# letitiabanana/PnP-OVSS

Measured on AMD Instinct MI355X. Metric: images/sec (336^2, drop_iter=4, blur+CRF), higher is better.
Workload: dtype bf16x3

## Files before the change

pnp-ovss_amd/csrc/engine.hip:

```cpp
#include <hip/hip_runtime.h>

#include <cmath>
#include <cstdarg>
#include <cstring>
#include <map>
#include <memory>
#include <string>
#include <utility>
#include <vector>

#include "../../include/pnp_hip.h"
#include "common.h"
#include "kernels.h"

using namespace pnp;

namespace {

struct Buf {
    void* p = nullptr;
    size_t bytes = 0;
};

struct Weight {
// ... 1569 lines not shown
        if (hist && p.d_gt) KCHK(e, confusion_hist(lab, p.d_gt, p.d_desc, p.d_label_off, hist, n_class, p.B, p.maxHW, s));
    }
    return PNP_OK;
}


extern "C" int pnp_get_buffer(pnp_engine* e, const char* name, void** d_ptr, size_t* bytes) {
    if (!e || !name || !d_ptr || !bytes) return PNP_ERR_ARG;
    const std::string n(name);
    const size_t B = e->c.max_batch, L = e->c.max_text_len;
    auto& p = e->post;
    auto set = [&](void* ptr, size_t b) { *d_ptr = ptr; *bytes = b; return PNP_OK; };
    if (n == "image_embeds") return set(e->emb32, B * e->N * (size_t)e->D * 4);
    if (n == "image_embeds_t") return set(e->embT.hi, B * e->N * (size_t)e->D * e->esz);
    if (n == "x") return set(e->x, B * e->N * (size_t)e->D * 4);
    if (n == "P") return set(e->ta[e->grad_layer >= 0 ? e->grad_layer : e->SL].Pc, B * e->nh * L * (size_t)e->Nst * 4);
    if (n == "dP") return set(e->dPc, B * e->nh * L * (size_t)e->Nst * 4);
    if (n == "text_hidden") return set(e->ta[e->TL - 1].h_out, B * L * (size_t)e->H * 4);
    if (n == "h_last") return set(e->ta[e->TL - 1].h_out, B * L * (size_t)e->H * 4);
    if (n == "dropped") return set(e->dropped, B * (size_t)e->PP);
    if (n == "P_last" && e->ta[e->TL - 1].Pc) return set(e->ta[e->TL - 1].Pc, B * e->nh * L * (size_t)e->Nst * 4);
    if (n == "Kt" && e->Kt) return set(e->Kt, (size_t)(e->TL - e->SL - 1) * e->H * B * e->Npad * e->esz);
    if (n == "Vt") return set(e->Vt, (size_t)e->TL * e->H * B * e->Npad * e->esz);
    if (n == "dq_xattn") return set(e->dqc, B * L * (size_t)e->H * e->esz);
    if (n == "dctx_xattn") return set(e->dctxc, B * L * (size_t)e->H * e->esz);
    if (p.reserved) {
        const size_t mk = (size_t)p.max_total_pix * p.maxK * 4;
        const size_t mq = (size_t)p.max_total_pix * p.maxKp * 4;
        if (n == "merged") return set(p.merged, (size_t)p.maxB * p.maxK * e->PP * 4);
        if (n == "maps") return set(p.maps_in_2 ? p.maps2 : p.maps, mk);
        if (n == "maps_pre_blur") return set(p.maps, mk);
        if (n == "unary") return set(p.unary, mq);
        if (n == "crf_q") return set(p.Q, mq);
        if (n == "crf_idbase_gauss") return set(p.lat[0].idbase, ((size_t)p.maxB + 1) * 4);
        if (n == "crf_idbase_bilateral") return set(p.lat[1].idbase, ((size_t)p.maxB + 1) * 4);
        if (n == "crf_norm_gauss") return set(p.norm[0], (size_t)p.max_total_pix * 4);
        if (n == "crf_norm_bilateral") return set(p.norm[1], (size_t)p.max_total_pix * 4);
        if (n == "crf_offset_gauss") return set(p.lat[0].offset, (size_t)p.max_total_pix * 3 * 4);
        if (n == "crf_offset_bilateral") return set(p.lat[1].offset, (size_t)p.max_total_pix * 6 * 4);
        if (n == "crf_nbr8_gauss") return set(p.lat[0].nbr8, (size_t)(p.lat[0].D1 / 2) * p.lat[0].cap * sizeof(CrfNbr8));
        if (n == "crf_nbr8_bilateral") return set(p.lat[1].nbr8, (size_t)(p.lat[1].D1 / 2) * p.lat[1].cap * sizeof(CrfNbr8));
    }
    return fail(e, PNP_ERR_ARG, "unknown buffer %s", name);
}

extern "C" size_t pnp_allocated_bytes(const pnp_engine* e) { return e ? e->alloc_bytes : 0; }

extern "C" int pnp_profile_enable(pnp_engine* e, int32_t on) {
    if (!e) return PNP_ERR_ARG;
    if (!e->gemm_prof) {
        if (!on) {
            e->crf_prof.on = false;
            return PNP_OK;
        }
        e->gemm_prof = new GemmProfile();
    }
    GemmProfile& pf = *e->gemm_prof;
    pf.on = on != 0;
    pf.period = on > 1 ? on : 1;
    pf.seq = 0;
    pf.used = 0;
    pf.launches = 0;
    pf.flops = 0;
    e->crf_prof.on = on != 0;
    e->crf_prof.used = 0;
    e->crf_prof.launches = 0;
    e->crf_prof.work = 0;
    e->crf_prof.lattice = 0;
    return PNP_OK;
}

extern "C" int pnp_profile_read_stage(pnp_engine* e, int32_t stage, int64_t* launches, double* work, double* ms) {
    if (!e || !launches || !work || !ms) return PNP_ERR_ARG;
    if (stage == 0) return pnp_profile_read(e, launches, work, ms);
    if (stage != 1 && stage != 2) return fail(e, PNP_ERR_ARG, "unknown profile stage %d", stage);
    auto& pf = e->crf_prof;
    double total = 0;
    for (int i = 0; i < pf.used; i++) {
        HIPCHK(e, hipEventSynchronize(pf.ev1[i]));
        float t = 0;
        HIPCHK(e, hipEventElapsedTime(&t, pf.ev0[i], pf.ev1[i]));
        total += t;
    }
    *launches = pf.launches;
    *work = stage == 1 ? pf.work : pf.lattice;
    *ms = total;
    return PNP_OK;
}

extern "C" int pnp_profile_read(pnp_engine* e, int64_t* launches, double* flops, double* ms) {
    if (!e || !launches || !flops || !ms) return PNP_ERR_ARG;
    if (!e->gemm_prof) {
        *launches = 0; *flops = 0; *ms = 0;
        return PNP_OK;
    }
    GemmProfile& pf = *e->gemm_prof;
    double total = 0;
    for (int i = 0; i < pf.used; i++) {
        HIPCHK(e, hipEventSynchronize(pf.ev1[i]));
        float t = 0;
        HIPCHK(e, hipEventElapsedTime(&t, pf.ev0[i], pf.ev1[i]));
        total += t;
    }
    *launches = pf.launches;
    *flops = pf.flops;
    *ms = total;
    return PNP_OK;
}

extern "C" int pnp_op_gemm(int32_t bf, const void* d_A, int32_t lda, const void* d_B, int32_t ldb, int32_t M, int32_t N,
                           int32_t K, const float* d_bias, const float* d_resid, int32_t ldr, float* d_out_f32, int32_t ldo,
                           int32_t gelu, void* stream) {
    GemmArgs g = G_(d_A, lda, d_B, ldb, M, N, K);
    g.bias = d_bias; g.resid = d_resid; g.ldr = ldr; g.out_f32 = d_out_f32; g.ldo = ldo;
    g.mode = gelu ? GEMM_EPI_GELU : GEMM_EPI_LINEAR;
    return gemm_nt(bf, g, (hipStream_t)stream);
}

extern "C" int pnp_op_gemm_ex(int32_t bf, const void* d_A, int32_t lda, const void* d_B, int32_t ldb, int32_t M, int32_t N,
                              int32_t K, const float* d_bias, const float* d_resid, int32_t ldr, float* d_out_f32, int32_t ldo,
                              void* d_out_t, int32_t ldo_t, int32_t mode, void* stream) {
    GemmArgs g = G_(d_A, lda, d_B, ldb, M, N, K);
    g.bias = d_bias; g.resid = d_resid; g.ldr = ldr; g.out_f32 = d_out_f32; g.ldo = ldo; g.out_t = d_out_t; g.ldo_t = ldo_t;
    g.mode = mode ? GEMM_EPI_GELU : GEMM_EPI_LINEAR;
    return gemm_nt(bf, g, (hipStream_t)stream);
}

extern "C" int pnp_op_split(const float* d_in, void* d_hi, void* d_lo, int64_t n, void* stream) {
    if (!d_in || !d_hi || !d_lo || n <= 0) return PNP_ERR_ARG;
    return split_f32(d_in, d_hi, d_lo, (size_t)n, (hipStream_t)stream);
}

extern "C" int pnp_op_gemm_x3(const void* d_A_hi, const void* d_A_lo, int32_t lda, const void* d_B_hi, const void* d_B_lo,
                              int32_t ldb, int32_t M, int32_t N, int32_t K, const float* d_bias, int32_t bias_on_rows,
                              const float* d_resid, int32_t ldr, float* d_out_f32, int32_t ldo, void* d_out_hi, void* d_out_lo,
                              int32_t ldo_t, int32_t gelu, int32_t col_div, int32_t col_pad, void* stream) {
    if (!d_A_hi || !d_A_lo || !d_B_hi || !d_B_lo) return PNP_ERR_ARG;
    GemmArgs g = G_(d_A_hi, lda, d_B_hi, ldb, M, N, K);
    g.A_lo = d_A_lo; g.B_lo = d_B_lo;
    g.bias = d_bias; g.bias_on_rows = bias_on_rows; g.resid = d_resid; g.ldr = ldr; g.out_f32 = d_out_f32; g.ldo = ldo;
    g.out_t = d_out_hi; g.out_lo = d_out_lo; g.ldo_t = ldo_t; g.col_div = col_div; g.col_pad = col_pad;
    g.mode = gelu ? GEMM_EPI_GELU : GEMM_EPI_LINEAR;
    g.sk = streamk_mode() ? streamk_ws_default() : nullptr;
    return gemm_nt(1, g, (hipStream_t)stream);
}

extern "C" int pnp_set_tuning(const char* key, int32_t value) {
    if (!key) return PNP_ERR_ARG;
    if (!strcmp(key, "streamk")) {
        if (value < 0 || value > 2) return PNP_ERR_ARG;
        set_streamk_mode(value);
        return PNP_OK;
    }
    if (!strcmp(key, "text_rows")) {
        if (value < 0 || value > 4) return PNP_ERR_ARG;
        set_text_rows(value);
        return PNP_OK;
    }
    return PNP_ERR_ARG;
}

extern "C" int pnp_streamk_status(pnp_engine* e, int64_t* launches, uint32_t* gave_up) {
    if (!launches || !gave_up) return PNP_ERR_ARG;
    StreamKWs* ws = e ? &e->sk_ws : streamk_ws_default();
    *launches = ws ? ws->launches : 0;
    *gave_up = 0;
    if (!ws || !ws->part) return PNP_OK;
    if (e) HIPCHK(e, hipSetDevice(e->c.device));
    if (hipDeviceSynchronize() != hipSuccess) return PNP_ERR_HIP;
    return streamk_ws_timeouts(ws, gave_up);
}

extern "C" int pnp_op_gemm_x3a(const float* d_A, int32_t lda, const void* d_B_hi, const void* d_B_lo, int32_t ldb, int32_t M,
                               int32_t N, int32_t K, const float* d_bias, const float* d_resid, int32_t ldr, float* d_out_f32,
                               int32_t ldo, int32_t mode, float* d_aux, int32_t ld_aux, void* stream) {
    if (!d_A || !d_B_hi || !d_B_lo || !d_out_f32 || mode < 0 || mode > 2) return PNP_ERR_ARG;
    GemmArgs g = G_(d_A, lda, d_B_hi, ldb, M, N, K);
    g.B_lo = d_B_lo; g.a_f32 = 1;
    g.bias = d_bias; g.resid = d_resid; g.ldr = ldr; g.out_f32 = d_out_f32; g.ldo = ldo;
    g.mode = mode; g.aux = d_aux; g.ld_aux = ld_aux;
    return gemm_nt(0, g, (hipStream_t)stream);
}

extern "C" int pnp_op_gemm_tokcols(int32_t bf, const void* d_A, int32_t lda, const void* d_B, int32_t ldb, int32_t M, int32_t N,
                                   int32_t K, const float* d_bias_rows, void* d_out_t, int32_t ldo_t, int32_t col_div,
                                   int32_t col_pad, void* stream) {
    if (!d_out_t || col_div < 0 || (col_div > 0 && col_pad < col_div)) return PNP_ERR_ARG;
    GemmArgs g = G_(d_A, lda, d_B, ldb, M, N, K);
    g.bias = d_bias_rows; g.bias_on_rows = 1; g.out_t = d_out_t; g.ldo_t = ldo_t; g.col_div = col_div; g.col_pad = col_pad;
    return gemm_nt(bf, g, (hipStream_t)stream);
}

extern "C" int pnp_op_gemm_args(int32_t bf, const void* d_A, int32_t lda, const void* d_B, int32_t ldb, int32_t M, int32_t N,
                                int32_t K, const float* d_bias, int32_t bias_on_rows, const float* d_resid, int32_t ldr,
                                float* d_out_f32, int32_t ldo, void* d_out_t, int32_t ldo_t, int32_t mode, float* d_aux,
                                int32_t ld_aux, int32_t row_div, int32_t col_div, int32_t col_pad, void* stream) {
    if (!d_A || !d_B || (!d_out_f32 && !d_out_t) || M <= 0 || N <= 0 || K <= 0 || lda < K || ldb < K) return PNP_ERR_ARG;
    if (mode < 0 || mode > 2 || (mode == GEMM_EPI_GELU_GRAD && !d_aux)) return PNP_ERR_ARG;
    if (row_div < 0 || col_div < 0 || (col_div > 0 && col_pad < col_div)) return PNP_ERR_ARG;
    GemmArgs g = G_(d_A, lda, d_B, ldb, M, N, K);
    g.bias = d_bias; g.bias_on_rows = bias_on_rows ? 1 : 0; g.resid = d_resid; g.ldr = ldr;
    g.out_f32 = d_out_f32; g.ldo = ldo; g.out_t = d_out_t; g.ldo_t = ldo_t;
    g.mode = mode; g.aux = d_aux; g.ld_aux = ld_aux; g.row_div = row_div; g.col_div = col_div; g.col_pad = col_pad;
    return gemm_nt(bf ? 1 : 0, g, (hipStream_t)stream);
}

extern "C" int pnp_op_vit_attention(int32_t bf, const void* d_qk, int32_t ld_qk, int32_t D, const void* d_vt, int32_t ld_vt,
                                    int32_t n_pad, void* d_ctx, int32_t B, int32_t heads, int32_t N, float scale, void* stream) {
    if (!d_qk || !d_vt || !d_ctx || B <= 0 || heads <= 0 || N <= 0) return PNP_ERR_ARG;
    return vit_attention(bf, d_qk, ld_qk, D, d_vt, ld_vt, n_pad, d_ctx, B, heads, N, scale, (hipStream_t)stream);
}

extern "C" int pnp_op_vit_attention_x3(const void* d_qkv_hi, const void* d_qkv_lo, int32_t ld_qkv, int32_t D, void* d_ctx_hi,
                                       void* d_ctx_lo, int32_t B, int32_t heads, int32_t N, float scale, void* stream) {
    if (B <= 0 || heads <= 0 || N <= 0 || ld_qkv < 3 * D) return PNP_ERR_ARG;
    return vit_attention_x3(d_qkv_hi, d_qkv_lo, ld_qkv, D, d_ctx_hi, d_ctx_lo, B, heads, N, scale, (hipStream_t)stream);
}

extern "C" int pnp_op_layernorm(const float* d_x, const float* d_w, const float* d_b, float eps, int32_t rows, int32_t D,
                                float* d_y, void* stream) {
    return layernorm(0, d_x, d_w, d_b, eps, rows, D, d_y, nullptr, nullptr, nullptr, (hipStream_t)stream);
}

extern "C" int pnp_op_xattn(int32_t bf16, int32_t mode, const void* d_nat, int32_t ld_nat, const void* d_tr, int32_t ld_tr,
                            int32_t n_pad, const void* d_x, int32_t ldx, void* d_out, int32_t ldo, float* d_probs,
                            int32_t n_stride, int32_t B, int32_t L, int32_t N, int32_t heads, void* stream) {
    if (!d_nat || !d_x || !d_probs || mode < 0 || mode > 2 || (mode != 2 && (!d_tr || !d_out))) return PNP_ERR_ARG;
    if (B <= 0 || L <= 0 || N <= 0 || heads <= 0) return PNP_ERR_ARG;
    return xattn(bf16, mode, d_nat, ld_nat, d_tr, ld_tr, n_pad, d_x, ldx, d_out, ldo, d_probs, n_stride, B, L, N, heads,
                 (hipStream_t)stream);
}

extern "C" int pnp_op_text_self_attn(int32_t bf16, const void* d_qkv, const int64_t* d_mask, int32_t ld_mask, void* d_ctx,
                                     float* d_probs, float* d_scratch, int32_t B, int32_t L, int32_t H, void* stream) {
    if (!d_qkv || !d_mask || !d_ctx || B <= 0 || L <= 0 || H <= 0 || ld_mask < L) return PNP_ERR_ARG;
    return text_self_attn(bf16, d_qkv, d_mask, ld_mask, d_ctx, d_probs, d_scratch, B, L, H, (hipStream_t)stream);
}

extern "C" int pnp_op_text_self_attn_bwd(int32_t bf16, const void* d_qkv, const float* d_dctx, const float* d_probs,
                                         float* d_ds_scratch, void* d_dqkv, int32_t B, int32_t L, int32_t H, void* stream) {
    if (!d_qkv || !d_dctx || !d_probs || !d_ds_scratch || !d_dqkv || B <= 0 || L <= 0 || H <= 0) return PNP_ERR_ARG;
    return text_self_attn_bwd(bf16, d_qkv, d_dctx, d_probs, d_ds_scratch, d_dqkv, B, L, H, (hipStream_t)stream);
}

extern "C" int pnp_op_layernorm_ex(int32_t bf16, const float* d_x, const float* d_w, const float* d_b, float eps, int32_t rows,
                                   int32_t D, float* d_y, void* d_yt, void* d_yt_lo, float* d_xhat, float* d_rstd, void* stream) {
    if (!d_x || !d_w || !d_b || rows <= 0 || D <= 0 || (d_yt_lo && !d_yt)) return PNP_ERR_ARG;
    return layernorm(bf16, d_x, d_w, d_b, eps, rows, D, d_y, d_yt, d_xhat, d_rstd, (hipStream_t)stream, d_yt_lo);
}

extern "C" int pnp_op_layernorm_bwd(int32_t bf16, const float* d_dy, const float* d_w, const float* d_xhat, const float* d_rstd,
                                    int32_t rows, int32_t D, float* d_dx, void* d_dxt, void* stream) {
    if (!d_dy || !d_w || !d_xhat || !d_rstd || rows <= 0 || D <= 0) return PNP_ERR_ARG;
    return layernorm_bwd(bf16, d_dy, d_w, d_xhat, d_rstd, rows, D, d_dx, d_dxt, (hipStream_t)stream);
}

extern "C" int pnp_op_text_embed(const int64_t* d_ids, int32_t ld_ids, const float* d_word, const float* d_pos, float* d_out,
                                 int32_t B, int32_t L, int32_t H, int32_t enc_id, int32_t vocab, void* stream) {
    if (!d_ids || !d_word || !d_pos || !d_out || B <= 0 || L <= 0 || H <= 0 || H % 4 || vocab <= 0 || ld_ids < L || enc_id >= vocab)
        return PNP_ERR_ARG;
    return text_embed(d_ids, ld_ids, d_word, d_pos, d_out, B, L, H, enc_id, vocab, (hipStream_t)stream);
}

extern "C" int pnp_op_itm_head(const float* d_hlast, const float* d_w, const float* d_bias, float* d_logits, int32_t B, int32_t L,
                               int32_t H, void* stream) {
    if (!d_hlast || !d_w || !d_bias || !d_logits || B <= 0 || L <= 0 || H <= 0) return PNP_ERR_ARG;
    return itm_head(d_hlast, d_w, d_bias, d_logits, B, L, H, (hipStream_t)stream);
}

extern "C" int pnp_op_itm_grad_seed(const float* d_w, float* d_dh, int32_t B, int32_t L, int32_t H, void* stream) {
    if (!d_w || !d_dh || B <= 0 || L <= 0 || H <= 0) return PNP_ERR_ARG;
    return itm_grad_seed(d_w, d_dh, B, L, H, (hipStream_t)stream);
}

extern "C" int pnp_op_patchify(int32_t bf16, const float* d_img, const uint8_t* d_dropped, void* d_out, int32_t B, int32_t S,
                               int32_t P, void* stream) {
    if (!d_img || !d_out || B <= 0 || P <= 0 || S != P * 16) return PNP_ERR_ARG;
    return patchify(bf16, d_img, d_dropped, d_out, B, S, P, (hipStream_t)stream);
}

extern "C" int pnp_op_cls_rows(const float* d_cls, const float* d_pos, float* d_x, int32_t B, int32_t N, int32_t D, void* stream) {
    if (!d_cls || !d_pos || !d_x || B <= 0 || N <= 0 || D <= 0) return PNP_ERR_ARG;
    return cls_rows(d_cls, d_pos, d_x, B, N, D, (hipStream_t)stream);
}

extern "C" int pnp_dbg_gemm_stamps(uint64_t* host_out, int32_t max_blocks) {
    return gemm_read_stamps((unsigned long long*)host_out, max_blocks);
}

extern "C" int pnp_preprocess_images(const uint8_t* d_rgb, const pnp_pre_image* d_desc, int32_t B, int32_t S, int32_t max_H,
                                     const int32_t* d_coef, uint8_t* d_tmp, const float* mean3, const float* std3,
                                     float* d_out, void* stream) {
    if (!d_rgb || !d_desc || !d_coef || !d_tmp || !mean3 || !std3 || !d_out) return PNP_ERR_ARG;
    static_assert(sizeof(pnp_pre_image) == 40, "pnp_pre_image layout is part of the ABI");
    return preprocess_images(d_rgb, d_desc, B, S, max_H, d_coef, d_tmp, mean3, std3, d_out, (hipStream_t)stream);
}

extern "C" int pnp_jpeg_decode(const uint8_t* d_data, const pnp_jpeg_image* d_images, const pnp_jpeg_tables* d_tables,
                               const pnp_jpeg_segment* d_segments, int32_t n_images, int32_t n_segments, uint8_t* d_clean,
                               int32_t* d_seg_bits, int16_t* d_coef, int64_t coef_elems, uint8_t* d_planes, uint8_t* d_rgb,
                               int32_t max_blocks_per_image, int32_t max_pixels_per_image, int32_t* d_err, void* stream) {
    if (!d_data || !d_images || !d_tables || !d_segments || !d_clean || !d_seg_bits || !d_coef || !d_planes || !d_rgb || !d_err ||
        coef_elems <= 0)
        return PNP_ERR_ARG;
    static_assert(sizeof(pnp_jpeg_image) == sizeof(JpegImage) && sizeof(pnp_jpeg_tables) == sizeof(JpegTables) &&
                      sizeof(pnp_jpeg_segment) == sizeof(JpegSegment), "JPEG descriptor layouts are part of the ABI");
// ... 33 lines not shown
```

pnp-ovss_amd/csrc/kernels.h:

```cpp
#pragma once
#include <hip/hip_runtime.h>
#include <stdint.h>
#include <stddef.h>
#include "gemm.h"

namespace pnp {

struct PostDesc {
    int H, W, K, C, has_bg, pix0;
    int Kp;
    int G, Kg;
    size_t off;
    size_t qoff;
    size_t voff[2];
};

struct alignas(16) CrfEntry {
    uint32_t pixel;
    float w;
    float nr;
    uint32_t pad;
};

struct alignas(16) CrfNbr8 {
    int ia, id;
    int pa, pd;
    int aa, ad;
    int da, dd;
};

struct CrfLattice {
    int D1;
    int which;
    size_t cap;
    float* bary;
    uint32_t* vals;
    CrfEntry* ent;
    int* offset;
    int* seg_start;
    int* seg_lo;
    int* seg_hi;
    uint64_t* ukeys;
    int* idbase;
    int* n1;
    int* n2;
    CrfNbr8* nbr8;
};

int patchify(int bf, const float* img, const uint8_t* dropped, void* out, int B, int S, int P, hipStream_t s);
int cls_rows(const float* cls, const float* pos, float* x, int B, int N, int D, hipStream_t s);
int layernorm(int bf, const float* x, const float* w, const float* b, float eps, int rows, int D, float* y, void* yt,
              float* xhat, float* rstd, hipStream_t s, void* yt_lo = nullptr);
int vit_attention(int bf, const void* qk, int ld_qk, int D, const void* vt, int ld_vt, int Npad, void* ctx, int B,
                  int H, int N, float scale, hipStream_t s, void* ctx_lo = nullptr);

int vit_attention_x3(const void* qkv_hi, const void* qkv_lo, int ld_qk, int D, void* ctx_hi, void* ctx_lo, int B, int H, int N,
                     float scale, hipStream_t s);

int text_embed(const int64_t* ids, int ld_ids, const float* word, const float* pos, float* out, int B, int L, int H,
               int enc_id, int vocab, hipStream_t s);
int text_self_attn(int bf, const void* qkv, const int64_t* mask, int ld_mask, void* ctx, float* probs, float* scratch, int B, int L,
                   int H, hipStream_t s);
void set_text_rows(int n);
int text_self_attn_bwd(int bf, const void* qkv, const float* dctx, const float* probs, float* ds_scratch, void* dqkv,
                       int B, int L, int H, hipStream_t s);
int xattn(int bf, int mode, const void* a1, int ld1, const void* a2t, int ld2, int Npad, const void* x, int ldx,
          void* out, int ldo, float* pbuf, int Nst, int B, int L, int N, int nheads, hipStream_t s);
int layernorm_bwd(int bf, const float* dy, const float* w, const float* xhat, const float* rstd, int rows, int D,
                  float* dx, void* dxt, hipStream_t s);
int itm_head(const float* hlast, const float* w, const float* bias, float* logits, int B, int L, int H, hipStream_t s);
int itm_grad_seed(const float* w, float* dh, int B, int L, int H, hipStream_t s);
int cast_f32(int bf, const float* in, void* out, size_t n, hipStream_t s);
int split_f32(const float* in, void* hi, void* lo, size_t n, hipStream_t s);

int l2_normalize_rows(float* x, int rows, int E, float eps, hipStream_t s);
int itc_similarity(const float* img, const float* txt, float* sim, int B, int T, int E, hipStream_t s);
int cast_rows_bf16(const float* in, int ld_in, void* out, int rows, int K, hipStream_t s);

int gradcam_gather(const float* P, const float* dP, const int64_t* mask, int ld_mask, float* out, int B, int nheads,
                   int head, int L, int Nst, int PP, hipStream_t s);
int drop_step(const float* G, float* g0, float* agg, uint8_t* dropped, int32_t* picks, int iter, int B, int T, int PP,
              int npick, int max_picks, hipStream_t s);
int merge_tokens(const float* src, const int32_t* cls_off, const int32_t* tok_idx, const int32_t* cls_div,
                 const int32_t* img_cls_off, float* out, int B, int T, int PP, int Cmax, hipStream_t s);
int threshold_maps(const float* merged, const int32_t* img_cls_off, float* out, float threshold, int B, int PP, int Cmax,
                   hipStream_t s);
int upsample_maps(const float* src, const PostDesc* desc, float* maps, int B, int P, int Cmax, int maxHW, hipStream_t s);
int minmax_normalize(float* maps, const PostDesc* desc, float* stats, int B, int Kmax, int maxHW, int class_channels_only,
                     hipStream_t s);
int background_channel(float* maps, const PostDesc* desc, int B, int maxHW, hipStream_t s);
int blur_maps(const float* in, float* tmp, float* out, const PostDesc* desc, const double* wts, const int32_t* wt_off,
              int B, int Kmax, int maxH, int maxW, int max_radius, hipStream_t s);
int preprocess_images(const uint8_t* rgb, const void* desc, int B, int S, int max_H, const int32_t* coef, uint8_t* tmp,
                      const float* mean3, const float* std3, float* out, hipStream_t s);
int unary_from_maps(const float* maps, const PostDesc* desc, float* unary, int B, int maxHW, int max_kp, int group, hipStream_t s);
int argmax_remap(const float* q, const PostDesc* desc, const int32_t* lut, int lut_stride, uint8_t* labels,
                 const size_t* label_off, int pixel_major, int group, int B, int maxHW, hipStream_t s);
int confusion_hist(const uint8_t* labels, const float* gt, const PostDesc* desc, const size_t* label_off,
                   unsigned long long* hist, int n_class, int B, int maxHW, hipStream_t s);

struct JpegImage {
    int64_t data_off;
    int64_t coef_off[3];
    int64_t plane_off[3];
    int64_t rgb_off;
    int32_t data_len, H, W, ncomp, hmax, vmax, mcux, mcuy;
    int32_t h[3], v[3], tq[3], td[3], ta[3], bx[3], by[3];
    int32_t tab, pad[2];
};
struct JpegTables {
    uint8_t counts[4][16];
    uint8_t vals[4][256];
    int32_t quant[4][64];
};
struct JpegSegment {
    int64_t byte_off;
    int64_t clean_off;
    int32_t image, mcu0, nmcu;
    int32_t raw_len;
    int32_t clean_cap;
    int32_t sub_bits;
    int32_t pad[2];
};
int jpeg_decode(const uint8_t* d_data, const JpegImage* d_imgs, const JpegTables* d_tabs, const JpegSegment* d_segs, int n_images,
                int n_segments, uint8_t* d_clean, int* d_seg_bits, int16_t* d_coef, size_t coef_elems, uint8_t* d_planes, uint8_t* d_rgb,
                int max_blocks, int max_pixels, int* d_err, hipStream_t s);

size_t sort_temp_bytes(size_t n);
int radix_sort_pairs(uint64_t* keys_in, uint64_t* keys_out, uint32_t* vals_in, uint32_t* vals_out, size_t n, int begin_bit, int end_bit,
                     const size_t* seg_off, int nseg, void* temp, size_t temp_bytes, hipStream_t s);
int device_scan_i32(const int* in, int* out, size_t n, bool inclusive, void* temp, size_t temp_bytes, hipStream_t s);
size_t crf_sort_temp_bytes(size_t max_entries, int max_images);
int crf_build_lattice(int D, const CrfLattice& L, const PostDesc* d_imgs, const PostDesc* h_imgs, const uint8_t* d_rgb, float sxy, float srgb,
                      int B, size_t ent_total, int max_pixels,
                      uint64_t* keys_a, uint64_t* keys_b, uint32_t* vals_a, int* head, int* incl, int* n1k, int* n2k,
                      void* temp, size_t temp_bytes, int* d_range_err, int* h_range_err, int* h_points, hipStream_t s);
int crf_lattice_norm(const CrfLattice& L, const PostDesc* d_imgs, int B, int max_pixels, size_t ent_total, float* va, float* vb,
                     float* norm_out, hipStream_t s);
int crf_filter(const CrfLattice& L, const PostDesc* d_imgs, int img0, int nimg, const float* Q,
               float* va, float* vb, const float** result, int max_kp, hipStream_t s);
struct CrfLabelOut {
    uint8_t* lab[2] = {nullptr, nullptr};
    const int32_t* lut = nullptr;
    int lut_stride = 0;
    const size_t* label_off = nullptr;
};
int crf_update(const CrfLattice& Lg, const CrfLattice& Lb, const PostDesc* d_imgs, int img0, int nimg, const float* vg,
               const float* vb, const float* norm_g, const float* norm_b, const float* unary, float* Q, float w_g,
               float w_b, int pairwise, int max_pixels, int max_kp, int groups, hipStream_t s, const CrfLabelOut& labels = CrfLabelOut());

}
```

pnp-ovss_amd/csrc/vit_kernels.hip:

```cpp
#include <stdlib.h>

#include "common.h"
#include "kernels.h"

namespace pnp {

template <typename T>
__global__ void patchify_kernel(const float* __restrict__ img, const uint8_t* __restrict__ dropped,
                                T* __restrict__ out, int B, int S, int P) {
    const int idx = blockIdx.x * blockDim.x + threadIdx.x;
    const int total = B * P * P * 3 * 16;
    if (idx >= total) return;
    const int i = idx & 15;
    const int c = (idx >> 4) % 3;
    const int m = idx / 48;
    const int b = m / (P * P), p = m - b * P * P;
    const int py = p / P, px = p - py * P;
    T* o = out + (size_t)m * 768 + c * 256 + i * 16;
    const bool drop = dropped && dropped[m];
    const float* src = img + (((size_t)b * 3 + c) * S + (py * 16 + i)) * S + px * 16;
#pragma unroll
    for (int v = 0; v < 4; v++) {
        f32x4 x = drop ? f32x4{0.f, 0.f, 0.f, 0.f} : *reinterpret_cast<const f32x4*>(src + v * 4);
#pragma unroll
// ... 219 lines not shown
    const int l32 = lane & 31, hi = lane >> 5;
    const int b = blockIdx.z, h = blockIdx.y;
    const size_t row0 = (size_t)b * N;
    const int qw = blockIdx.x * nwaves + wave;
    int qrow = qw * 32 + l32;
    const bool q_valid = qw < nqw && qrow < N;
    qrow = qrow < N ? qrow : N - 1;

    bf16x8 fq[4];
    {
        const bf16* qp = qk + (row0 + qrow) * ld_qk + h * 64 + hi * 8;
#pragma unroll
        for (int ks = 0; ks < 4; ks++) fq[ks] = *reinterpret_cast<const bf16x8*>(qp + ks * 16);
    }

    const char* kbase = reinterpret_cast<const char*>(qk + row0 * ld_qk + D + h * 64);
    const char* vbase = reinterpret_cast<const char*>(vt + row0 * ld_vt + h * 64);
    const int prow = lane >> 3, pc = lane & 7;
    auto issue_tile = [&](int t) {
        char* dst = ring[t & 1];
        for (int p = wave; p < 16; p += nwaves) {
            const int row = (p & 7) * 8 + prow;
            const int sc = pc ^ ((row >> 1) & 7);
            int key = t * 64 + row;
            key = key < N ? key : N - 1;
            const char* src = p < 8 ? kbase + (size_t)key * ld_qk * 2 + sc * 16 : vbase + (size_t)key * ld_vt * 2 + sc * 16;
            __builtin_amdgcn_global_load_lds((const __attribute__((address_space(1))) void*)src,
                                             (__attribute__((address_space(3))) void*)(dst + p * 1024), 16, 0, 0);
        }
    };

    f32x16 o[2];
#pragma unroll
    for (int i = 0; i < 2; i++)
#pragma unroll
        for (int e = 0; e < 16; e++) o[i][e] = 0.f;
    float m_run = -INFINITY, l_run = 0.f;
    const float c = scale * 1.4426950408889634f;
    const int sw = (l32 >> 1) & 7;
    const int ntiles = (N + 63) / 64;

    issue_tile(0);
    for (int t = 0; t < ntiles; t++) {
        asm volatile("s_waitcnt vmcnt(0)" ::: "memory");
        __builtin_amdgcn_s_barrier();
        if (t + 1 < ntiles) issue_tile(t + 1);
        const char* Ks = ring[t & 1];
        const char* Vs = Ks + TILE;

        bf16x8 fk[2][4];
#pragma unroll
        for (int kt = 0; kt < 2; kt++)
#pragma unroll
            for (int ks = 0; ks < 4; ks++)
                fk[kt][ks] = *reinterpret_cast<const bf16x8*>(Ks + (kt * 32 + l32) * ROWB + (((ks * 2 + hi) ^ sw) << 4));
        f32x16 s[2];
        const f32x16 zero16 = {0.f, 0.f, 0.f, 0.f, 0.f, 0.f, 0.f, 0.f, 0.f, 0.f, 0.f, 0.f, 0.f, 0.f, 0.f, 0.f};
#pragma unroll
        for (int kt = 0; kt < 2; kt++) {
            s[kt] = __builtin_amdgcn_mfma_f32_32x32x16_bf16(fk[kt][0], fq[0], zero16, 0, 0, 0);
#pragma unroll
            for (int ks = 1; ks < 4; ks++) s[kt] = __builtin_amdgcn_mfma_f32_32x32x16_bf16(fk[kt][ks], fq[ks], s[kt], 0, 0, 0);
        }
        if (t == ntiles - 1 && (N & 63)) {
#pragma unroll
            for (int kt = 0; kt < 2; kt++)
#pragma unroll
                for (int e = 0; e < 16; e++) {
                    const int key = t * 64 + kt * 32 + (e >> 2) * 8 + hi * 4 + (e & 3);
                    if (key >= N) s[kt][e] = -INFINITY;
                }
        }
        float mx;
        asm("v_max3_f32 %0, %1, %2, %3" : "=v"(mx) : "v"(s[0][0]), "v"(s[0][1]), "v"(s[0][2]));
#pragma unroll
        for (int e = 3; e + 1 < 16; e += 2) asm("v_max3_f32 %0, %1, %2, %3" : "=v"(mx) : "v"(mx), "v"(s[0][e]), "v"(s[0][e + 1]));
        asm("v_max3_f32 %0, %1, %2, %3" : "=v"(mx) : "v"(mx), "v"(s[0][15]), "v"(s[1][0]));
#pragma unroll
        for (int e = 1; e + 1 < 16; e += 2) asm("v_max3_f32 %0, %1, %2, %3" : "=v"(mx) : "v"(mx), "v"(s[1][e]), "v"(s[1][e + 1]));
        asm("v_max3_f32 %0, %1, %2, %3" : "=v"(mx) : "v"(mx), "v"(s[1][15]), "v"(m_run));
        const float m_new = fmaxf(mx, __shfl_xor(mx, 32, 64));
        {
            const float alpha = __builtin_amdgcn_exp2f((m_run - m_new) * c);
#pragma unroll
            for (int i = 0; i < 2; i++) o[i] *= alpha;
            l_run *= alpha;
            m_run = m_new;
        }
        const float mc = -m_run * c;
        bf16x8 fp[4];
#pragma unroll
        for (int kt = 0; kt < 2; kt++)
#pragma unroll
            for (int e = 0; e < 16; e++) {
                const float p = __builtin_amdgcn_exp2f(fmaf(s[kt][e], c, mc));
                l_run += p;
                fp[kt * 2 + (e >> 3)][e & 7] = (bf16)p;
            }
        const int grp_d = ((lane >> 4) & 1) * 16, tq = (lane >> 2) & 3, tp = lane & 3;
#pragma unroll
        for (int j = 0; j < 4; j++)
#pragma unroll
            for (int dt = 0; dt < 2; dt++) {
                typedef __attribute__((ext_vector_type(4))) short s16x4;
                s16x4 part[2];
#pragma unroll
                for (int u = 0; u < 2; u++) {
                    const int key = 16 * j + 8 * u + 4 * hi + tq;
                    const int col = dt * 32 + grp_d + 4 * tp;
                    const char* a = Vs + key * ROWB + ((((col >> 3)) ^ ((key >> 1) & 7)) << 4) + (col & 7) * 2;
                    part[u] = __builtin_amdgcn_ds_read_tr16_b64_v4i16((__attribute__((address_space(3))) s16x4*)a);
                }
                const bf16x4 lo = __builtin_bit_cast(bf16x4, part[0]), hh = __builtin_bit_cast(bf16x4, part[1]);
                const bf16x8 fv = {lo[0], lo[1], lo[2], lo[3], hh[0], hh[1], hh[2], hh[3]};
                o[dt] = __builtin_amdgcn_mfma_f32_32x32x16_bf16(fv, fp[j], o[dt], 0, 0, 0);
            }
    }
    l_run += __shfl_xor(l_run, 32, 64);
    if (q_valid) {
        const float inv = 1.0f / l_run;
        bf16* op = ctx + (row0 + qrow) * D + h * 64 + hi * 4;
#pragma unroll
        for (int dt = 0; dt < 2; dt++)
#pragma unroll
            for (int g4 = 0; g4 < 4; g4++) {
                const bf16x4 pk = {(bf16)(o[dt][g4 * 4] * inv), (bf16)(o[dt][g4 * 4 + 1] * inv), (bf16)(o[dt][g4 * 4 + 2] * inv),
                                   (bf16)(o[dt][g4 * 4 + 3] * inv)};
                *reinterpret_cast<bf16x4*>(op + dt * 32 + g4 * 8) = pk;
            }
    }
}

#ifdef PNP_DEV
__device__ unsigned long long* g_attn_stamps = nullptr;
__device__ int g_attn_ablate = 0;
extern "C" int pnp_dev_attn_ablate(int on) {
    return hipMemcpyToSymbol(HIP_SYMBOL(g_attn_ablate), &on, sizeof(on)) == hipSuccess ? PNP_OK : PNP_ERR_HIP;
}
extern "C" int pnp_dev_attn_stamps(unsigned long long* d_buf) {
    return hipMemcpyToSymbol(HIP_SYMBOL(g_attn_stamps), &d_buf, sizeof(d_buf)) == hipSuccess ? PNP_OK : PNP_ERR_HIP;
}
#define PNP_ATTN_STAMP(k)                                                                                       \
    do {                                                                                                        \
        if (stamps && lane == 0) {                                                                              \
            __builtin_amdgcn_sched_barrier(0);                                                                  \
            stamps[((size_t)wave * ntiles + t) * 6 + (k)] = __builtin_readcyclecounter();                       \
            __builtin_amdgcn_sched_barrier(0);                                                                  \
        }                                                                                                       \
    } while (0)
#else
#define PNP_ATTN_STAMP(k) do {} while (0)
#endif

__global__ __launch_bounds__(768) void vit_attn32_x3_kernel(const bf16* __restrict__ qk, const bf16* __restrict__ qk_lo, int ld_qk, int D,
                                                            const bf16* __restrict__ vt, const bf16* __restrict__ vt_lo, int ld_vt,
                                                            bf16* __restrict__ ctx, bf16* __restrict__ ctx_lo, int N, float scale, int nqw) {
    constexpr int ROWB = 128, TILE = 64 * ROWB;
    __shared__ __attribute__((aligned(16))) char ring[2][4 * TILE];

    const int tid = threadIdx.x, lane = tid & 63, wave = __builtin_amdgcn_readfirstlane(tid >> 6);
    const int nwaves = blockDim.x >> 6;
    const int l32 = lane & 31, hi = lane >> 5;
    const int b = blockIdx.z, h = blockIdx.y;
    const size_t row0 = (size_t)b * N;
    const int qw = blockIdx.x * nwaves + wave;
    int qrow = qw * 32 + l32;
    const bool q_valid = qw < nqw && qrow < N;
    qrow = qrow < N ? qrow : N - 1;

    bf16x8 fq[4], fql[4];
    {
        const size_t off = (row0 + qrow) * ld_qk + h * 64 + hi * 8;
#pragma unroll
        for (int ks = 0; ks < 4; ks++) {
            fq[ks] = *reinterpret_cast<const bf16x8*>(qk + off + ks * 16);
            fql[ks] = *reinterpret_cast<const bf16x8*>(qk_lo + off + ks * 16);
        }
    }
    const size_t koff = (row0 * ld_qk + D + h * 64) * 2, voff = (row0 * ld_vt + h * 64) * 2;
    const uint64_t k0 = reinterpret_cast<uint64_t>(qk) + koff;
    const uint64_t d_klo = reinterpret_cast<uint64_t>(qk_lo) + koff - k0;
    const uint64_t d_v = reinterpret_cast<uint64_t>(vt) + voff - k0;
    const uint64_t d_vlo = reinterpret_cast<uint64_t>(vt_lo) + voff - k0;
    const int prow = lane >> 3, pc = lane & 7;
    const uint32_t sc_even = (uint32_t)(pc ^ ((prow >> 1) & 7)) << 4, sc_odd = (uint32_t)(pc ^ ((4 + (prow >> 1)) & 7)) << 4;
    auto issue_tile = [&](int t) {
        for (int p = wave; p < 32; p += nwaves) {
            const uint64_t m_v = 0ull - (uint64_t)((p >> 3) & 1), m_lo = 0ull - (uint64_t)(p >> 4);
            const uint64_t d = (m_v & m_lo & d_vlo) | (m_v & ~m_lo & d_v) | (~m_v & m_lo & d_klo);
            const uint32_t ld2 = ((uint32_t)ld_qk + ((uint32_t)m_v & (uint32_t)(ld_vt - ld_qk))) * 2u;
            int rs = t * 64 + (p & 7) * 8;
#ifdef PNP_DEV
            if (g_attn_ablate) rs = (p & 7) * 8;
#endif
            rs = rs < N - 1 ? rs : N - 1;
            const char* const sbase = reinterpret_cast<const char*>(k0 + d + (uint64_t)((uint32_t)rs * ld2));
            int lr = rs + prow;
            lr = (lr < N ? lr : N - 1) - rs;
            const uint32_t loff = (uint32_t)lr * ld2 + ((p & 1) ? sc_odd : sc_even);
            const uint32_t lds = (uint32_t)(uintptr_t)(__attribute__((address_space(3))) char*)(ring[t & 1] + p * 1024);
            const uint64_t sb = reinterpret_cast<uint64_t>(sbase);
            const uint64_t sbu = ((uint64_t)(uint32_t)__builtin_amdgcn_readfirstlane((int)(sb >> 32)) << 32) |
                                 (uint32_t)__builtin_amdgcn_readfirstlane((int)(uint32_t)sb);
            asm volatile("s_mov_b32 m0, %2\n\ts_nop 0\n\tglobal_load_lds_dwordx4 %0, %1" ::"v"(loff), "s"(sbu),
                         "s"(__builtin_amdgcn_readfirstlane((int)lds))
                         : "memory");
        }
    };

    f32x16 o[2];
#pragma unroll
    for (int i = 0; i < 2; i++)
#pragma unroll
        for (int e = 0; e < 16; e++) o[i][e] = 0.f;
    float m_run = -INFINITY, l_run = 0.f;
    const float c = scale * 1.4426950408889634f;
    const int sw = (l32 >> 1) & 7;
    const int ntiles = (N + 63) / 64;

#ifdef PNP_DEV
    unsigned long long* const stamps = (blockIdx.x | blockIdx.y | blockIdx.z) == 0 ? g_attn_stamps : nullptr;
#endif
    issue_tile(0);
    for (int t = 0; t < ntiles; t++) {
        PNP_ATTN_STAMP(0);
        asm volatile("s_waitcnt vmcnt(0)" ::: "memory");
        __builtin_amdgcn_s_barrier();
        PNP_ATTN_STAMP(1);
        if (t + 1 < ntiles) issue_tile(t + 1);
        PNP_ATTN_STAMP(2);
        const char* Ks = ring[t & 1];
        const char* Vs = Ks + TILE;
        const char* Kl = Ks + 2 * TILE;
        const char* Vl = Ks + 3 * TILE;

        f32x16 s[2];
        const f32x16 zero16 = {0.f, 0.f, 0.f, 0.f, 0.f, 0.f, 0.f, 0.f, 0.f, 0.f, 0.f, 0.f, 0.f, 0.f, 0.f, 0.f};
#pragma unroll
        for (int kt = 0; kt < 2; kt++) {
            s[kt] = zero16;
#pragma unroll
            for (int ks = 0; ks < 4; ks++) {
                const int a = (kt * 32 + l32) * ROWB + (((ks * 2 + hi) ^ sw) << 4);
                const bf16x8 kl = *reinterpret_cast<const bf16x8*>(Kl + a);
                const bf16x8 kh = *reinterpret_cast<const bf16x8*>(Ks + a);
                s[kt] = __builtin_amdgcn_mfma_f32_32x32x16_bf16(kl, fq[ks], s[kt], 0, 0, 0);
                s[kt] = __builtin_amdgcn_mfma_f32_32x32x16_bf16(kh, fql[ks], s[kt], 0, 0, 0);
                s[kt] = __builtin_amdgcn_mfma_f32_32x32x16_bf16(kh, fq[ks], s[kt], 0, 0, 0);
            }
        }
        PNP_ATTN_STAMP(3);
        if (t == ntiles - 1 && (N & 63)) {
#pragma unroll
            for (int kt = 0; kt < 2; kt++)
#pragma unroll
                for (int e = 0; e < 16; e++) {
                    const int key = t * 64 + kt * 32 + (e >> 2) * 8 + hi * 4 + (e & 3);
                    if (key >= N) s[kt][e] = -INFINITY;
                }
        }
        float mx = m_run;
#pragma unroll
        for (int kt = 0; kt < 2; kt++)
#pragma unroll
            for (int e = 0; e < 16; e++) mx = fmaxf(mx, s[kt][e]);
        const float m_new = fmaxf(mx, __shfl_xor(mx, 32, 64));
        {
            const float alpha = __builtin_amdgcn_exp2f((m_run - m_new) * c);
#pragma unroll
            for (int i = 0; i < 2; i++) o[i] *= alpha;
            l_run *= alpha;
            m_run = m_new;
        }
        const float mc = -m_run * c;
        bf16x8 fp[4], fpl[4];
#pragma unroll
        for (int kt = 0; kt < 2; kt++)
#pragma unroll
            for (int e = 0; e < 16; e++) {
                const float p = __builtin_amdgcn_exp2f(fmaf(s[kt][e], c, mc));
                l_run += p;
                const bf16 ph = (bf16)p;
                fp[kt * 2 + (e >> 3)][e & 7] = ph;
                fpl[kt * 2 + (e >> 3)][e & 7] = (bf16)(p - (float)ph);
            }
        PNP_ATTN_STAMP(4);
        const int grp_d = ((lane >> 4) & 1) * 16, tq = (lane >> 2) & 3, tp = lane & 3;
#pragma unroll
        for (int j = 0; j < 4; j++)
#pragma unroll
            for (int dt = 0; dt < 2; dt++) {
                typedef __attribute__((ext_vector_type(4))) short s16x4;
                bf16x8 fv[2];
#pragma unroll
                for (int part = 0; part < 2; part++) {
                    const char* V = part ? Vl : Vs;
                    s16x4 pr[2];
#pragma unroll
                    for (int u = 0; u < 2; u++) {
                        const int key = 16 * j + 8 * u + 4 * hi + tq;
                        const int col = dt * 32 + grp_d + 4 * tp;
                        const char* a = V + key * ROWB + ((((col >> 3)) ^ ((key >> 1) & 7)) << 4) + (col & 7) * 2;
                        pr[u] = __builtin_amdgcn_ds_read_tr16_b64_v4i16((__attribute__((address_space(3))) s16x4*)a);
                    }
                    const bf16x4 lo = __builtin_bit_cast(bf16x4, pr[0]), hh = __builtin_bit_cast(bf16x4, pr[1]);
                    fv[part] = bf16x8{lo[0], lo[1], lo[2], lo[3], hh[0], hh[1], hh[2], hh[3]};
                }
                o[dt] = __builtin_amdgcn_mfma_f32_32x32x16_bf16(fv[1], fp[j], o[dt], 0, 0, 0);
                o[dt] = __builtin_amdgcn_mfma_f32_32x32x16_bf16(fv[0], fpl[j], o[dt], 0, 0, 0);
                o[dt] = __builtin_amdgcn_mfma_f32_32x32x16_bf16(fv[0], fp[j], o[dt], 0, 0, 0);
            }
        PNP_ATTN_STAMP(5);
    }
    l_run += __shfl_xor(l_run, 32, 64);
    if (q_valid) {
        const float inv = 1.0f / l_run;
        const size_t off = (row0 + qrow) * D + h * 64 + hi * 4;
#pragma unroll
        for (int dt = 0; dt < 2; dt++)
#pragma unroll
            for (int g4 = 0; g4 < 4; g4++) {
                bf16x4 ph, pl;
#pragma unroll
                for (int e = 0; e < 4; e++) {
                    const float v = o[dt][g4 * 4 + e] * inv;
                    ph[e] = (bf16)v;
                    pl[e] = (bf16)(v - (float)ph[e]);
                }
                *reinterpret_cast<bf16x4*>(ctx + off + dt * 32 + g4 * 8) = ph;
                *reinterpret_cast<bf16x4*>(ctx_lo + off + dt * 32 + g4 * 8) = pl;
            }
    }
}

int vit_attention(int bf, const void* qk, int ld_qk, int D, const void* vt, int ld_vt, int Npad, void* ctx, int B,
                  int H, int N, float scale, hipStream_t s, void* ctx_lo) {
    if (D != H * 64 || Npad % 64 || Npad < N) return PNP_ERR_ARG;
    if (bf) {
        if (ctx_lo) return PNP_ERR_ARG;
        const int nqw = (N + 31) / 32;
        const int max_wpb = 8;
        const int nblk = (nqw + max_wpb - 1) / max_wpb, wpb = (nqw + nblk - 1) / nblk;
        hipLaunchKernelGGL(vit_attn32_kernel, dim3(nblk, H, B), dim3(wpb * 64), 0, s, (const bf16*)qk, ld_qk, D,
                           (const bf16*)vt, ld_vt, Npad, (bf16*)ctx, N, scale, nqw);
        return hipGetLastError() == hipSuccess ? PNP_OK : PNP_ERR_HIP;
    }
    dim3 grid((N + 63) / 64, H, B);
    hipLaunchKernelGGL((vit_attn_kernel<float>), grid, dim3(256), 0, s, (const float*)qk, ld_qk, D, (const float*)vt, ld_vt,
                       Npad, ctx_lo ? nullptr : (float*)ctx, N, scale, ctx_lo ? (bf16*)ctx : nullptr, (bf16*)ctx_lo);
    return hipGetLastError() == hipSuccess ? PNP_OK : PNP_ERR_HIP;
}

int vit_attention_x3(const void* qkv_hi, const void* qkv_lo, int ld_qk, int D, void* ctx_hi, void* ctx_lo, int B, int H, int N,
                     float scale, hipStream_t s) {
    if (D != H * 64 || !qkv_hi || !qkv_lo || !ctx_hi || !ctx_lo) return PNP_ERR_ARG;
    const int nqw = (N + 31) / 32;
    int max_wpb = nqw > 24 ? 12 : 8;
#ifdef PNP_DEV
    if (getenv("PNP_ATTN_WPB")) max_wpb = atoi(getenv("PNP_ATTN_WPB"));
#endif
    const int nblk = (nqw + max_wpb - 1) / max_wpb, wpb = (nqw + nblk - 1) / nblk;
    const bf16 *qh = (const bf16*)qkv_hi, *ql = (const bf16*)qkv_lo;
    hipLaunchKernelGGL(vit_attn32_x3_kernel, dim3(nblk, H, B), dim3(wpb * 64), 0, s, qh, ql, ld_qk, D, qh + 2 * D, ql + 2 * D, ld_qk,
                       (bf16*)ctx_hi, (bf16*)ctx_lo, N, scale, nqw);
    return hipGetLastError() == hipSuccess ? PNP_OK : PNP_ERR_HIP;
}

int patchify(int bf, const float* img, const uint8_t* dropped, void* out, int B, int S, int P, hipStream_t s) {
    const int total = B * P * P * 48;
    const int nb = (total + 255) / 256;
    if (bf) hipLaunchKernelGGL((patchify_kernel<bf16>), dim3(nb), dim3(256), 0, s, img, dropped, (bf16*)out, B, S, P);
    else hipLaunchKernelGGL((patchify_kernel<float>), dim3(nb), dim3(256), 0, s, img, dropped, (float*)out, B, S, P);
    return hipGetLastError() == hipSuccess ? PNP_OK : PNP_ERR_HIP;
}

int cls_rows(const float* cls, const float* pos, float* x, int B, int N, int D, hipStream_t s) {
    hipLaunchKernelGGL(cls_rows_kernel, dim3((B * D + 255) / 256), dim3(256), 0, s, cls, pos, x, B, N, D);
    return hipGetLastError() == hipSuccess ? PNP_OK : PNP_ERR_HIP;
}

int layernorm(int bf, const float* x, const float* w, const float* b, float eps, int rows, int D, float* y, void* yt,
              float* xhat, float* rstd, hipStream_t s, void* yt_lo) {
    if (D > 1024 || D % 4) return PNP_ERR_ARG;
    if (yt_lo && !bf) return PNP_ERR_ARG;
    const int nb = (rows + 3) / 4;
    if (bf) hipLaunchKernelGGL((layernorm_kernel<bf16>), dim3(nb), dim3(256), 0, s, x, w, b, eps, rows, D, y, (bf16*)yt, xhat, rstd, (bf16*)yt_lo);
    else hipLaunchKernelGGL((layernorm_kernel<float>), dim3(nb), dim3(256), 0, s, x, w, b, eps, rows, D, y, (float*)yt, xhat, rstd, (bf16*)nullptr);
    return hipGetLastError() == hipSuccess ? PNP_OK : PNP_ERR_HIP;
}

}
```

Baseline: 221.0.

## Template ViT x3 attention on ring slot size and precompute DMA offsets

Templates the split-bf16 ViT attention kernel on the number of keys per ring slot (64 or 128), so one barrier and wait can cover two 64-key sub-tiles. The shared-memory ring becomes dynamic, with the size chosen per instantiation. K and V are now addressed from one fused qkv base, and per-wave DMA offsets are precomputed, removing the per-issue mask arithmetic and readfirstlane work. The default stays 64, so the main gain on the default path is the cheaper address setup; the 128 mode, reachable through a tuning key, doubles LDS use and may reduce occupancy.

```diff
diff --git a/pnp-ovss_amd/csrc/engine.hip b/pnp-ovss_amd/csrc/engine.hip
--- a/pnp-ovss_amd/csrc/engine.hip
+++ b/pnp-ovss_amd/csrc/engine.hip
@@ -1745,6 +1745,11 @@
         set_streamk_mode(value);
         return PNP_OK;
     }
+    if (!strcmp(key, "attn_slot_keys")) {
+        if (value != 64 && value != 128) return PNP_ERR_ARG;
+        set_attn_slot_keys(value);
+        return PNP_OK;
+    }
     if (!strcmp(key, "text_rows")) {
         if (value < 0 || value > 4) return PNP_ERR_ARG;
         set_text_rows(value);
diff --git a/pnp-ovss_amd/csrc/kernels.h b/pnp-ovss_amd/csrc/kernels.h
--- a/pnp-ovss_amd/csrc/kernels.h
+++ b/pnp-ovss_amd/csrc/kernels.h
@@ -56,6 +56,7 @@
 
 int vit_attention_x3(const void* qkv_hi, const void* qkv_lo, int ld_qk, int D, void* ctx_hi, void* ctx_lo, int B, int H, int N,
                      float scale, hipStream_t s);
+void set_attn_slot_keys(int keys);
 
 int text_embed(const int64_t* ids, int ld_ids, const float* word, const float* pos, float* out, int B, int L, int H,
                int enc_id, int vocab, hipStream_t s);
diff --git a/pnp-ovss_amd/csrc/vit_kernels.hip b/pnp-ovss_amd/csrc/vit_kernels.hip
--- a/pnp-ovss_amd/csrc/vit_kernels.hip
+++ b/pnp-ovss_amd/csrc/vit_kernels.hip
@@ -395,11 +395,15 @@
 #define PNP_ATTN_STAMP(k) do {} while (0)
 #endif
 
-__global__ __launch_bounds__(768) void vit_attn32_x3_kernel(const bf16* __restrict__ qk, const bf16* __restrict__ qk_lo, int ld_qk, int D,
-                                                            const bf16* __restrict__ vt, const bf16* __restrict__ vt_lo, int ld_vt,
+template <int SLOT_KEYS>
+__global__ __launch_bounds__(768) void vit_attn32_x3_kernel(const bf16* __restrict__ qkv, const bf16* __restrict__ qkv_lo, int ld, int D,
                                                             bf16* __restrict__ ctx, bf16* __restrict__ ctx_lo, int N, float scale, int nqw) {
     constexpr int ROWB = 128, TILE = 64 * ROWB;
-    __shared__ __attribute__((aligned(16))) char ring[2][4 * TILE];
+    constexpr int SUB = SLOT_KEYS / 64, SLOT_BYTES = SUB * 4 * TILE;
+    constexpr int NPAIR = 16 * SUB;
+    constexpr int MAXP = SUB == 1 ? 3 : 5;
+    static_assert(SLOT_KEYS == 64 || SLOT_KEYS == 128, "ring slot: one or two 64-key sub-tiles");
+    extern __shared__ __attribute__((aligned(16))) char ring[];
 
     const int tid = threadIdx.x, lane = tid & 63, wave = __builtin_amdgcn_readfirstlane(tid >> 6);
     const int nwaves = blockDim.x >> 6;
@@ -413,42 +417,72 @@
 
     bf16x8 fq[4], fql[4];
     {
-        const size_t off = (row0 + qrow) * ld_qk + h * 64 + hi * 8;
+        const size_t off = (row0 + qrow) * ld + h * 64 + hi * 8;
 #pragma unroll
         for (int ks = 0; ks < 4; ks++) {
-            fq[ks] = *reinterpret_cast<const bf16x8*>(qk + off + ks * 16);
-            fql[ks] = *reinterpret_cast<const bf16x8*>(qk_lo + off + ks * 16);
-        }
-    }
-    const size_t koff = (row0 * ld_qk + D + h * 64) * 2, voff = (row0 * ld_vt + h * 64) * 2;
-    const uint64_t k0 = reinterpret_cast<uint64_t>(qk) + koff;
-    const uint64_t d_klo = reinterpret_cast<uint64_t>(qk_lo) + koff - k0;
-    const uint64_t d_v = reinterpret_cast<uint64_t>(vt) + voff - k0;
-    const uint64_t d_vlo = reinterpret_cast<uint64_t>(vt_lo) + voff - k0;
+            fq[ks] = *reinterpret_cast<const bf16x8*>(qkv + off + ks * 16);
+            fql[ks] = *reinterpret_cast<const bf16x8*>(qkv_lo + off + ks * 16);
+        }
+    }
+    const size_t koff = (row0 * ld + D + h * 64) * 2;
+    auto scalar64 = [](uint64_t v) {
+        return ((uint64_t)(uint32_t)__builtin_amdgcn_readfirstlane((int)(v >> 32)) << 32) |
+               (uint32_t)__builtin_amdgcn_readfirstlane((int)(uint32_t)v);
+    };
+    const uint64_t base_hi = scalar64(reinterpret_cast<uint64_t>(qkv) + koff), base_lo = scalar64(reinterpret_cast<uint64_t>(qkv_lo) + koff);
     const int prow = lane >> 3, pc = lane & 7;
+    const uint32_t ld2 = (uint32_t)ld * 2u;
     const uint32_t sc_even = (uint32_t)(pc ^ ((prow >> 1) & 7)) << 4, sc_odd = (uint32_t)(pc ^ ((4 + (prow >> 1)) & 7)) << 4;
-    auto issue_tile = [&](int t) {
-        for (int p = wave; p < 32; p += nwaves) {
-            const uint64_t m_v = 0ull - (uint64_t)((p >> 3) & 1), m_lo = 0ull - (uint64_t)(p >> 4);
-            const uint64_t d = (m_v & m_lo & d_vlo) | (m_v & ~m_lo & d_v) | (~m_v & m_lo & d_klo);
-            const uint32_t ld2 = ((uint32_t)ld_qk + ((uint32_t)m_v & (uint32_t)(ld_vt - ld_qk))) * 2u;
-            int rs = t * 64 + (p & 7) * 8;
+    const int nslots = (N + SLOT_KEYS - 1) / SLOT_KEYS;
+    const uint32_t lds_ring = (uint32_t)(uintptr_t)(__attribute__((address_space(3))) char*)ring;
+    auto dma = [&](uint32_t off, uint64_t sbase, uint32_t lds) {
+        asm volatile("s_mov_b32 m0, %2\n\ts_nop 0\n\tglobal_load_lds_dwordx4 %0, %1" ::"v"(off), "s"(sbase),
+                     "s"(__builtin_amdgcn_readfirstlane((int)lds))
+                     : "memory");
+    };
+    auto pair_col = [&](int j) { return (uint32_t)((j >> 3) & 1) * (uint32_t)D * 2u; };
+    auto pair_lds = [&](int j) { return (uint32_t)(j + (j & ~15)) * 1024u; };
+    uint32_t poff[MAXP], plds[MAXP];
+#pragma unroll
+    for (int i = 0; i < MAXP; i++) {
+        const int j = wave + i * nwaves;
+        poff[i] = pair_col(j) + (uint32_t)((j >> 4) * 64 + (j & 7) * 8) * ld2;
+        plds[i] = pair_lds(j);
+    }
+    const int npair = (NPAIR - wave + nwaves - 1) / nwaves;
+    const uint32_t loff_even = (uint32_t)prow * ld2 + sc_even, loff_odd = (uint32_t)prow * ld2 + sc_odd;
+    const uint32_t loff_first = (wave & 1) ? loff_odd : loff_even, loff_flip = (nwaves & 1) ? (loff_even ^ loff_odd) : 0u;
+    auto issue_pair = [&](int j, int s, int key0) {
+        if (s * SLOT_KEYS + (j >> 4) * 64 >= N) return;
+        int rs = key0 + (j >> 4) * 64 + (j & 7) * 8;
+        rs = rs < N - 1 ? rs : N - 1;
+        int lr = rs + prow;
+        lr = (lr < N ? lr : N - 1) - rs;
+        const uint32_t off = pair_col(j) + (uint32_t)rs * ld2 + (uint32_t)lr * ld2 + ((j & 1) ? sc_odd : sc_even);
+        const uint32_t lds = lds_ring + (uint32_t)((s & 1) * SLOT_BYTES) + pair_lds(j);
+        dma(off, base_hi, lds);
+        dma(off, base_lo, lds + 16 * 1024);
+    };
+    auto issue_tile = [&](int s) {
+        int key0 = s * SLOT_KEYS;
 #ifdef PNP_DEV
-            if (g_attn_ablate) rs = (p & 7) * 8;
+        if (g_attn_ablate) key0 = 0;
 #endif
-            rs = rs < N - 1 ? rs : N - 1;
-            const char* const sbase = reinterpret_cast<const char*>(k0 + d + (uint64_t)((uint32_t)rs * ld2));
-            int lr = rs + prow;
-            lr = (lr < N ? lr : N - 1) - rs;
-            const uint32_t loff = (uint32_t)lr * ld2 + ((p & 1) ? sc_odd : sc_even);
-            const uint32_t lds = (uint32_t)(uintptr_t)(__attribute__((address_space(3))) char*)(ring[t & 1] + p * 1024);
-            const uint64_t sb = reinterpret_cast<uint64_t>(sbase);
-            const uint64_t sbu = ((uint64_t)(uint32_t)__builtin_amdgcn_readfirstlane((int)(sb >> 32)) << 32) |
-                                 (uint32_t)__builtin_amdgcn_readfirstlane((int)(uint32_t)sb);
-            asm volatile("s_mov_b32 m0, %2\n\ts_nop 0\n\tglobal_load_lds_dwordx4 %0, %1" ::"v"(loff), "s"(sbu),
-                         "s"(__builtin_amdgcn_readfirstlane((int)lds))
-                         : "memory");
-        }
+        if (s == nslots - 1) {
+            for (int j = wave; j < NPAIR; j += nwaves) issue_pair(j, s, key0);
+            return;
+        }
+        const uint32_t adv = (uint32_t)key0 * ld2, lds_slot = lds_ring + (uint32_t)((s & 1) * SLOT_BYTES);
+        uint32_t loff = loff_first;
+#pragma unroll
+        for (int i = 0; i < MAXP; i++) {
+            if (i >= npair) break;
+            const uint32_t off = loff + (poff[i] + adv);
+            dma(off, base_hi, lds_slot + plds[i]);
+            dma(off, base_lo, lds_slot + plds[i] + 16 * 1024);
+            loff ^= loff_flip;
+        }
+        for (int j = wave + MAXP * nwaves; j < NPAIR; j += nwaves) issue_pair(j, s, key0);
     };
 
     f32x16 o[2];
@@ -465,14 +499,26 @@
     unsigned long long* const stamps = (blockIdx.x | blockIdx.y | blockIdx.z) == 0 ? g_attn_stamps : nullptr;
 #endif
     issue_tile(0);
-    for (int t = 0; t < ntiles; t++) {
+    for (int slot = 0; slot < nslots; slot++) {
+      {
+        [[maybe_unused]] const int t = slot * SUB;
         PNP_ATTN_STAMP(0);
         asm volatile("s_waitcnt vmcnt(0)" ::: "memory");
         __builtin_amdgcn_s_barrier();
         PNP_ATTN_STAMP(1);
-        if (t + 1 < ntiles) issue_tile(t + 1);
+        if (slot + 1 < nslots) issue_tile(slot + 1);
         PNP_ATTN_STAMP(2);
-        const char* Ks = ring[t & 1];
+      }
+#pragma unroll 1
+      for (int u = 0; u < SUB; u++) {
+        const int t = slot * SUB + u;
+        if (t >= ntiles) break;
+        if (u) {
+            PNP_ATTN_STAMP(0);
+            PNP_ATTN_STAMP(1);
+            PNP_ATTN_STAMP(2);
+        }
+        const char* Ks = ring + (slot & 1) * SLOT_BYTES + u * (4 * TILE);
         const char* Vs = Ks + TILE;
         const char* Kl = Ks + 2 * TILE;
         const char* Vl = Ks + 3 * TILE;
@@ -554,6 +600,7 @@
                 o[dt] = __builtin_amdgcn_mfma_f32_32x32x16_bf16(fv[0], fp[j], o[dt], 0, 0, 0);
             }
         PNP_ATTN_STAMP(5);
+      }
     }
     l_run += __shfl_xor(l_run, 32, 64);
     if (q_valid) {
@@ -594,6 +641,20 @@
     return hipGetLastError() == hipSuccess ? PNP_OK : PNP_ERR_HIP;
 }
 
+static std::atomic<int> g_attn_slot_keys{64};
+void set_attn_slot_keys(int keys) { g_attn_slot_keys.store(keys, std::memory_order_relaxed); }
+
+template <int SLOT_KEYS>
+static int launch_attn_x3(const bf16* qh, const bf16* ql, int ld_qk, int D, bf16* ctx_hi, bf16* ctx_lo, int B, int H, int N, float scale,
+                          int nblk, int wpb, int nqw, hipStream_t s) {
+    constexpr int smem = 2 * (SLOT_KEYS / 64) * 4 * 64 * 128;
+    static std::atomic<uint32_t> opted{0};
+    if (lds_opt_in(opted, reinterpret_cast<const void*>(vit_attn32_x3_kernel<SLOT_KEYS>), smem) != PNP_OK) return PNP_ERR_HIP;
+    hipLaunchKernelGGL((vit_attn32_x3_kernel<SLOT_KEYS>), dim3(nblk, H, B), dim3(wpb * 64), smem, s, qh, ql, ld_qk, D, ctx_hi, ctx_lo, N,
+                       scale, nqw);
+    return hipGetLastError() == hipSuccess ? PNP_OK : PNP_ERR_HIP;
+}
+
 int vit_attention_x3(const void* qkv_hi, const void* qkv_lo, int ld_qk, int D, void* ctx_hi, void* ctx_lo, int B, int H, int N,
                      float scale, hipStream_t s) {
     if (D != H * 64 || !qkv_hi || !qkv_lo || !ctx_hi || !ctx_lo) return PNP_ERR_ARG;
@@ -604,9 +665,9 @@
 #endif
     const int nblk = (nqw + max_wpb - 1) / max_wpb, wpb = (nqw + nblk - 1) / nblk;
     const bf16 *qh = (const bf16*)qkv_hi, *ql = (const bf16*)qkv_lo;
-    hipLaunchKernelGGL(vit_attn32_x3_kernel, dim3(nblk, H, B), dim3(wpb * 64), 0, s, qh, ql, ld_qk, D, qh + 2 * D, ql + 2 * D, ld_qk,
-                       (bf16*)ctx_hi, (bf16*)ctx_lo, N, scale, nqw);
-    return hipGetLastError() == hipSuccess ? PNP_OK : PNP_ERR_HIP;
+    if (g_attn_slot_keys.load(std::memory_order_relaxed) == 128)
+        return launch_attn_x3<128>(qh, ql, ld_qk, D, (bf16*)ctx_hi, (bf16*)ctx_lo, B, H, N, scale, nblk, wpb, nqw, s);
+    return launch_attn_x3<64>(qh, ql, ld_qk, D, (bf16*)ctx_hi, (bf16*)ctx_lo, B, H, N, scale, nblk, wpb, nqw, s);
 }
 
 int patchify(int bf, const float* img, const uint8_t* dropped, void* out, int B, int S, int P, hipStream_t s) {
```

New measurement: 222.1 (median of 6 runs). No clear change (+0.5%).
